# jinhan/tacotron2-vae

Hardware: AMD Instinct MI355X
Metric: mel-frames/s (train step, batch=6, 80-mel) (higher is better)
Workload: dtype f32; 1 GPU; configs[1]: Tacotron2-VAE fp32 train step (fwd+loss+bwd+clip+Adam), B=6/GPU fixed shape T_in=84 T_out=400, dropout on, random-init seed 1234; step_mode=hip-graph replay, decoder_forward=persistent, decoder_backward=persistent, startup_steps=43, global_batch=6, parallelism=dp1

## Files before the change

include/t2vae.h:

```cpp
#ifndef T2VAE_H
#define T2VAE_H
#include <stdint.h>
#ifdef __cplusplus
extern "C" {
#endif

#define T2V_OK 0
#define T2V_ERR_DIMS -1
#define T2V_ERR_ARG -2
#define T2V_ERR_LAUNCH -3

const char* t2v_version(void);
const char* t2v_last_error(void);

void t2v_set_phase_profile(unsigned long long* dev_buf32);
int t2v_stamp(unsigned long long* dev_buf, int slot, void* stream);
int t2v_debug_spin(int wgs, int microseconds, void* stream);

typedef struct t2v_step_params {
    uint64_t epoch;
    float lr;
    float bc1;
    float bc2s;
    float kl_weight;
// ... 165 lines not shown
    const float* proj_b;
    const float* prenet_w1;
} t2v_dec_persist_weights;
typedef struct t2v_dec_persist_bufs {
    const float* memory;
    const float* pm;
    const int32_t* lengths;
    const float* pre_first;
    float* MEL;
    float* GATE;
    float* AL;
    int32_t* stop_flag;
    void* exchange;
    uint32_t* err_word;
} t2v_dec_persist_bufs;
long t2v_decoder_persist_scratch_floats(int B, int t_end);
int t2v_decoder_persist_supported(int B, int T_in);
int t2v_decoder_infer_persistent(const t2v_dec_persist_weights* w, const t2v_dec_persist_bufs* s, int B, int T_in,
                                 int t_end, float gate_threshold, float p_prenet, uint64_t seed, void* stream);

typedef struct t2v_dec_items {
    int32_t* stop_item;
    const uint64_t* item_seeds;
} t2v_dec_items;
int t2v_decoder_infer_steps_items(const t2v_dec_weights* w, const t2v_dec_infer_bufs* s, int B, int T_in,
                                  int t_begin, int t_end, float gate_threshold, float p_prenet,
                                  int external_prenet, uint64_t seed, const t2v_dec_items* items, void* stream);
int t2v_decoder_infer_persistent_items(const t2v_dec_persist_weights* w, const t2v_dec_persist_bufs* s, int B, int T_in,
                                       int t_end, float gate_threshold, float p_prenet, uint64_t seed,
                                       const t2v_dec_items* items, void* stream);

int t2v_conv1d_stat_blocks(int B, int T, int Cin, int Cout, int KS);
int t2v_conv1d_stat_blocks_bf16(int B, int T, int Cin, int Cout, int KS);
int t2v_conv1d_fwd(const float* W, const float* X, const float* bias, float* Y, float* stat_part,
                   int B, int Cin, int T, int Cout, int KS, void* stream);
int t2v_conv1d_dw_scratch_floats(int B, int Cin, int T, int Cout, int KS);
int t2v_conv1d_bwd(const float* W, const float* X, const float* dY, float* dX, float* dW, float* Wt_scratch,
                   float* dw_scratch,
                   int B, int Cin, int T, int Cout, int KS, void* stream);
int t2v_conv1d_flip_weights(const float* const* W, float* const* Wt, const int* Cout, const int* Cin, int KS, int n,
                            void* stream);
int t2v_conv1d_fwd_bf16(const float* W, const float* X, const float* bias, float* Y, float* stat_part,
                        void* Wp_scratch, int B, int Cin, int T, int Cout, int KS, void* stream);
int t2v_conv1d_bwd_bf16(const float* W, const float* X, const float* dY, float* dX, float* dW,
                        void* Wp_scratch, float* dw_scratch, int B, int Cin, int T, int Cout, int KS, void* stream);

int t2v_bn_act_fwd(const float* y, const float* stat_part, int nblk, const float* gamma, const float* beta,
                   float* running_mean, float* running_var, float* mean_out, float* rstd_out, float* out,
                   int B, int M, int T, int act, int training, float p_drop, float momentum, float eps,
                   uint64_t seed, uint32_t rng_stream, uint32_t rng_t, void* stream);
int t2v_bn_act_fwd_len(const float* y, const float* gamma, const float* beta, const float* running_mean,
                       const float* running_var, float* out, const int32_t* lengths, int B, int M, int T, int act, float eps,
                       void* stream);
int t2v_bn_act_bwd(const float* y, const float* dout, const float* mean, const float* rstd,
                   const float* gamma, const float* beta, float* dy, float* dgamma, float* dbeta,
                   float* dconv_bias, int B, int M, int T, int act, float p_drop, uint64_t seed,
                   uint32_t rng_stream, uint32_t rng_t, void* stream);
int t2v_bn_act_bwd_eval(const float* y, const float* dout, const float* mean, const float* rstd,
                   const float* gamma, const float* beta, float* dy, float* dgamma, float* dbeta,
                   float* dconv_bias, int B, int M, int T, int act, float p_drop, uint64_t seed,
                   uint32_t rng_stream, uint32_t rng_t, void* stream);

int t2v_embedding_fwd(const long long* ids, const float* W, float* out_bct, int B, int T, int C, int n_symbols, void* stream);
int t2v_embedding_bwd(const long long* ids, const float* dy_bct, float* dW, int B, int T, int C, int n_symbols, void* stream);

int t2v_gemm_epilogue_bwd(const float* dy, const float* y, float* out, size_t n, float scale, void* stream);
// ... 198 lines not shown
```

tacotron2-vae_amd/csrc/conv_gemm.hip:

```cpp
#include <stdlib.h>
#include "t2v_common.h"
#include "t2v_kernels.h"
#include "t2v_coop.h"


#define CG_BM 64
#define CG_BN 64
#define CG_BK 32

struct ConvGemmArgs {
    const float* W;
    const float* X;
    const float* dY;
    const float* bias;
    float* Y;
    float* stat_part;
    int B, Cin, T, M, KS;
};

template <int MODE, int KS>
__global__ __launch_bounds__(256) void k_conv_gemm(ConvGemmArgs a) {
    __shared__ float As[2][CG_BK][CG_BM + 1];
    __shared__ float Bs[2][CG_BK][CG_BN + 1];
    __shared__ float red[2][CG_BM][2];
    const int tid = threadIdx.x, wave = tid >> 6, lane = tid & 63;
    const int wm = wave >> 1, wn = wave & 1;
    const int m0 = blockIdx.y * CG_BM, n0 = blockIdx.x * CG_BN;
    constexpr int P = KS >> 1;
    const int BT = a.B * a.T, CK = a.Cin * KS;
    const int Kdim = MODE == 0 ? CK : BT;
    const int Ndim = MODE == 0 ? BT : CK;

    constexpr int NE = CG_BM * CG_BK / 256;
    float ra[NE], rb[NE];
    int b_bb = 0, b_t = 0;
    bool b_nok = false;
// ... 95 lines not shown
                red[wn][ml][1] = q;
            }
        }
        __syncthreads();
        if (tid < CG_BM) {
            const int m = m0 + tid;
            if (m < a.M) {
                float* dst = a.stat_part + ((size_t)blockIdx.x * a.M + m) * 2;
                dst[0] = red[0][tid][0] + red[1][tid][0];
                dst[1] = red[0][tid][1] + red[1][tid][1];
            }
        }
    }
}

#define CT_BM 64
#define CT_AS 80
#define CT_KT 80

struct ConvTiledArgs {
    const float* W;
    const float* X;
    const float* dY;
    const float* bias;
    float* Y;
    float* stat_part;
    int B, Cin, T, M, tiles_per_item;
    unsigned long long* prof;
    float* ks_part;
    unsigned* ks_ctr;
};

template <int NTW>
__global__ __launch_bounds__(256) void k_conv5_fwd(ConvTiledArgs a) {
    constexpr int BN = 16 * NTW;
    constexpr int XW = BN + 4;
    constexpr int XS = BN == 32 ? 48 : BN <= 64 ? 80 : 112;
    constexpr int NX = (16 * XW + 255) / 256;
    __shared__ float As[2][CT_KT][CT_AS];
    __shared__ float Xs[2][16][XS];
    const int tid = threadIdx.x, wave = tid >> 6, lane = tid & 63;
    const int kq = lane >> 4, j = lane & 15;
    const int bb = blockIdx.x / a.tiles_per_item, t0 = (blockIdx.x % a.tiles_per_item) * BN;
    const int m0 = blockIdx.y * CT_BM;
    const int CK = a.Cin * 5;
    const int nkt_all = a.Cin / 16;
    const int kt0 = gridDim.z > 1 ? (int)blockIdx.z * (nkt_all / 2) : 0;
    const int nkt = gridDim.z > 1 ? (blockIdx.z == 0 ? nkt_all / 2 : nkt_all - nkt_all / 2) : nkt_all;

    const bool stamp = a.prof && tid == 0 && blockIdx.x == 0 && blockIdx.y == 0 && blockIdx.z == 0;
    if (stamp) { a.prof[0] = __builtin_readcyclecounter(); a.prof[2] = wall_clock64(); }
    float4 ra[5];
    float rx[NX];
    const int a_m = tid & 63, w4 = tid >> 6;
    const float* a_row = a.W + (size_t)min(m0 + a_m, a.M - 1) * CK + 4 * w4;
    int a_lds[20];
#pragma unroll
    for (int q = 0; q < 20; ++q) {
        const int k = 4 * w4 + 16 * (q >> 2) + (q & 3);
        const int c = k / 5, kx = k - 5 * c;
        a_lds[q] = (16 * kx + c) * CT_AS + a_m;
    }
    const float* x_item = a.X + (size_t)bb * a.Cin * a.T;
    int x_goff[NX], x_lds[NX];
    bool x_ok[NX];
#pragma unroll
// ... 35 lines not shown
    for (int q = 0; q < NSTORE; ++q) store_one(0, q);
    __syncthreads();
    for (int kt = 0; kt < nkt; ++kt) {
        const int buf = kt & 1;
        const int kn = min(kt + 1, nkt - 1);
        const float* ap = &As[buf][kq][16 * wave + j];
        const float* xp = &Xs[buf][kq][j];
        float av[2], bv[2][NTW];
        av[0] = ap[0];
#pragma unroll
        for (int n = 0; n < NTW; ++n) bv[0][n] = xp[16 * n];
#pragma unroll
        for (int s = 0; s < 20; ++s) {
            if (s < NLOAD) load_one(kn, s);
            if (s + 1 < 20) {
                av[(s + 1) & 1] = ap[4 * (s + 1) * CT_AS];
#pragma unroll
                for (int n = 0; n < NTW; ++n)
                    bv[(s + 1) & 1][n] = xp[4 * ((s + 1) & 3) * XS + 16 * n + ((s + 1) >> 2)];
            }
            __builtin_amdgcn_sched_barrier(0);
#pragma unroll
            for (int n = 0; n < NTW; ++n) acc[n] = mfma16x4(av[s & 1], bv[s & 1][n], acc[n]);
            __builtin_amdgcn_sched_barrier(0);
            if (s >= S_ST0) {
#pragma unroll
                for (int q = 3 * (s - S_ST0); q < 3 * (s - S_ST0) + 3; ++q) store_one(buf ^ 1, q);
                __builtin_amdgcn_sched_barrier(0);
            }
        }
        __syncthreads();
    }
    if (stamp) { a.prof[1] = __builtin_readcyclecounter(); a.prof[3] = wall_clock64(); }
    if (gridDim.z > 1) {
        const size_t tile = (size_t)blockIdx.y * gridDim.x + blockIdx.x, ntile = (size_t)gridDim.x * gridDim.y;
        float* mine = a.ks_part + ((blockIdx.z * ntile + tile) * 256 + tid) * (4 * NTW);
#pragma unroll
        for (int n = 0; n < NTW; ++n)
#pragma unroll
            for (int r = 0; r < 4; ++r) st_sc1(mine + 4 * n + r, acc[n][r]);
        __shared__ unsigned second_;
        asm volatile("s_waitcnt vmcnt(0)" ::: "memory");
        __syncthreads();
        if (tid == 0) second_ = __hip_atomic_fetch_add(a.ks_ctr + tile, 1u, __ATOMIC_RELAXED, __HIP_MEMORY_SCOPE_AGENT);
        __syncthreads();
        if (second_ == 0u) return;
        if (tid == 0) __hip_atomic_store(a.ks_ctr + tile, 0u, __ATOMIC_RELAXED, __HIP_MEMORY_SCOPE_AGENT);
        const float* other = a.ks_part + (((1 - blockIdx.z) * ntile + tile) * 256 + tid) * (4 * NTW);
        float o[NTW][4];
#pragma unroll
        for (int n = 0; n < NTW; ++n)
#pragma unroll
            for (int r = 0; r < 4; ++r) o[n][r] = ld_sc1(other + 4 * n + r);
#pragma unroll
        for (int n = 0; n < NTW; ++n)
#pragma unroll
            for (int r = 0; r < 4; ++r) acc[n][r] += o[n][r];
    }
    float psum[4] = {0.f, 0.f, 0.f, 0.f}, psq[4] = {0.f, 0.f, 0.f, 0.f};
#pragma unroll
    for (int r = 0; r < 4; ++r) {
        const int m = m0 + 16 * wave + 4 * kq + r;
        if (m < a.M) {
            const float bv = a.bias ? a.bias[m] : 0.f;
            float* yrow = a.Y + ((size_t)bb * a.M + m) * a.T;
#pragma unroll
            for (int n = 0; n < NTW; ++n) {
                const int t = t0 + 16 * n + j;
                if (t < a.T) {
                    const float v = acc[n][r] + bv;
                    yrow[t] = v;
                    psum[r] += v;
                    psq[r] = fmaf(v, v, psq[r]);
                }
            }
        }
    }
    if (a.stat_part) {
#pragma unroll
        for (int r = 0; r < 4; ++r) {
            const float s1 = row16_sum(psum[r]), s2 = row16_sum(psq[r]);
            const int m = m0 + 16 * wave + 4 * kq + r;
            if (j == 0 && m < a.M) {
                float* dst = a.stat_part + ((size_t)blockIdx.x * a.M + m) * 2;
                dst[0] = s1;
                dst[1] = s2;
            }
        }
    }
}

template <int BT>
__global__ __launch_bounds__(256) void k_conv5_dw(ConvTiledArgs a) {
    constexpr int XW = BT + 4;
    constexpr int XS = (BT == 80) ? 100 : 116;
    constexpr int NA = BT / 16;
    constexpr int NX = (16 * XW + 255) / 256;
    __shared__ float As[2][BT][CT_AS];
    __shared__ float Xs[2][16][XS];
    const int tid = threadIdx.x, wave = tid >> 6, lane = tid & 63;
    const int kq = lane >> 4, j = lane & 15;
    const int c0 = blockIdx.x * 16, m0 = blockIdx.y * CT_BM;
    const int CK = a.Cin * 5;
    const int tiles = (a.T + BT - 1) / BT, nkt_all = a.B * tiles;
    const int per = (nkt_all + gridDim.z - 1) / gridDim.z;
    const int kt_lo = blockIdx.z * per, kt_hi = min(nkt_all, kt_lo + per);
    const bool vec = (a.T & 3) == 0;

    float4 ra[NA];
    float rx[NX];
    const int a_m = tid & 63;
    const bool a_ok = m0 + a_m < a.M;
    auto load_tiles = [&](int kt) {
        const int bb = kt / tiles, t0 = (kt - bb * tiles) * BT;
        const float* arow = a.dY + ((size_t)bb * a.M + (a_ok ? m0 + a_m : 0)) * a.T;
#pragma unroll
        for (int i = 0; i < NA; ++i) {
            const int t = t0 + 4 * ((tid >> 6) + 4 * i);
            float4 v = make_float4(0.f, 0.f, 0.f, 0.f);
            if (a_ok) {
                if (vec) {
                    if (t < a.T) v = *(const float4*)(arow + t);
// ... 503 lines not shown
    for (int i = 0; i < 5; ++i) {
        const int bn = cands[i];
        const long wgs = (long)B * ((T + bn - 1) / bn) * ((M + CT_BM - 1) / CT_BM);
        const long cost = ((wgs + T2V_NWG - 1) / T2V_NWG) * (bn + 40);
        if (best_cost < 0 || cost < best_cost || (cost == best_cost && bn > best)) { best = bn; best_cost = cost; }
    }
    return best;
}
static inline int conv5_pick_bn_ks(int T, int B, int M, int Cin, int* ks) {
    static const int ksplit_on = getenv("T2V_CONV_KSPLIT") ? atoi(getenv("T2V_CONV_KSPLIT")) : 1;
    *ks = 1;
    const int bn1 = conv5_pick_bn(T, B, M);
    if (!ksplit_on || Cin < 256 || getenv("T2V_CONV_BN")) return bn1;
    const int cands[5] = {32, 48, 64, 80, 96};
    const long w1 = (long)B * ((T + bn1 - 1) / bn1) * ((M + CT_BM - 1) / CT_BM);
    long best_cost = 2 * ((w1 + T2V_NWG - 1) / T2V_NWG) * (bn1 + 40);
    int best = bn1;
    for (int i = 0; i < 5; ++i) {
        const int bn = cands[i];
        const long wgs = 2 * (long)B * ((T + bn - 1) / bn) * ((M + CT_BM - 1) / CT_BM);
        if (wgs > (ksplit_on == 2 ? 2 * T2V_NWG : T2V_NWG)) continue;
        const long cost = ((wgs + T2V_NWG - 1) / T2V_NWG) * ((bn + 40) + 16);
        if (cost < best_cost) { best = bn; best_cost = cost; *ks = 2; }
    }
    return best;
}
static inline bool conv5_tiled_ok(int Cin, int KS) { return KS == 5 && Cin % 16 == 0; }
bool t2v_conv5_x3_ok(int B, int Cin, int T, int Cout, int KS);
int t2v_conv5_x3_stat_blocks(int B, int T);
int t2v_conv5_x3_run(const float* W, const float* X, const float* bias, float* Y, float* stat_part, int B, int Cin, int T, int M,
                     hipStream_t stream, int np);
bool t2v_conv5_planes_bf16_ok(int B, int Cin, int T, int Cout, int KS);

static void launch_conv5_fwd(const float* W, const float* X, const float* bias, float* Y, float* stat_part, int B,
                             int Cin, int T, int M, hipStream_t stream) {
    int ks = 1;
    const int BN = conv5_pick_bn_ks(T, B, M, Cin, &ks);
    ConvTiledArgs a;
    a.W = W; a.X = X; a.dY = nullptr; a.bias = bias; a.Y = Y; a.stat_part = stat_part;
    a.B = B; a.Cin = Cin; a.T = T; a.M = M; a.tiles_per_item = (T + BN - 1) / BN;
    a.prof = g_t2v_prof;
    a.ks_part = nullptr; a.ks_ctr = nullptr;
    dim3 grid(B * a.tiles_per_item, (M + CT_BM - 1) / CT_BM);
    const long ntile = (long)grid.x * grid.y;
    if (ks == 2) {
        const size_t pf = (size_t)2 * ntile * 256 * 4 * (BN / 16);
        a.ks_part = conv_ks_scratch(pf);
        a.ks_ctr = a.ks_part ? t2v_arrival_counters((int)ntile) : nullptr;
        if (a.ks_part && a.ks_ctr) grid.z = 2; else a.ks_part = nullptr;
    }
    if (BN == 32) k_conv5_fwd<2><<<grid, 256, 0, stream>>>(a);
    else if (BN == 48) k_conv5_fwd<3><<<grid, 256, 0, stream>>>(a);
    else if (BN == 64) k_conv5_fwd<4><<<grid, 256, 0, stream>>>(a);
    else if (BN == 80) k_conv5_fwd<5><<<grid, 256, 0, stream>>>(a);
    else k_conv5_fwd<6><<<grid, 256, 0, stream>>>(a);
}

static void launch_conv5_fwd_bf16(const float* W, int flipT, unsigned short* Wp, const float* X, const float* bias,
                                  float* Y, float* stat_part, int B, int Cin, int T, int M, int W_M, int W_Cin,
                                  hipStream_t stream) {
    const size_t n = (size_t)W_M * W_Cin * 5;
    k_conv5_pack_bf16<<<(unsigned)((n + 255) / 256), 256, 0, stream>>>(W, Wp, W_M, W_Cin, flipT);
    int ks_unused = 1;
    const int BN = conv5_pick_bn_ks(T, B, M, Cin, &ks_unused);
    ConvBf16Args a;
    a.Wp = Wp; a.X = X; a.bias = bias; a.Y = Y; a.stat_part = stat_part;
    a.B = B; a.Cin = Cin; a.T = T; a.M = M; a.tiles_per_item = (T + BN - 1) / BN;
    dim3 grid(B * a.tiles_per_item, (M + CT_BM - 1) / CT_BM);
    static const int k32 = getenv("T2V_CONV_BF16_K32") ? atoi(getenv("T2V_CONV_BF16_K32")) : 1;
    if (k32 && Cin % 32 == 0) {
        if (BN == 32) k_conv5_fwd_bf16k32<2><<<grid, 256, 0, stream>>>(a);
        else if (BN == 48) k_conv5_fwd_bf16k32<3><<<grid, 256, 0, stream>>>(a);
        else if (BN == 64) k_conv5_fwd_bf16k32<4><<<grid, 256, 0, stream>>>(a);
        else if (BN == 80) k_conv5_fwd_bf16k32<5><<<grid, 256, 0, stream>>>(a);
        else k_conv5_fwd_bf16k32<6><<<grid, 256, 0, stream>>>(a);
        return;
    }
    if (BN == 32) k_conv5_fwd_bf16<2><<<grid, 256, 0, stream>>>(a);
    else if (BN == 48) k_conv5_fwd_bf16<3><<<grid, 256, 0, stream>>>(a);
    else if (BN == 64) k_conv5_fwd_bf16<4><<<grid, 256, 0, stream>>>(a);
    else if (BN == 80) k_conv5_fwd_bf16<5><<<grid, 256, 0, stream>>>(a);
    else k_conv5_fwd_bf16<6><<<grid, 256, 0, stream>>>(a);
// ... 177 lines not shown
```

tacotron2-vae_amd/csrc/t2v_x3.h:

```cpp
#pragma once
#include "t2v_common.h"

__device__ __forceinline__ void t2v_split8(const float (&v)[8], uint4& p0, uint4& p1, uint4& p2) {
    unsigned q0[4], q1[4], q2[4];
#pragma unroll
    for (int c = 0; c < 4; ++c) {
        const float x = v[2 * c], y = v[2 * c + 1];
        const unsigned h = t2v_pack_bf16x2(x, y);
        const float r1x = x - __uint_as_float(h << 16), r1y = y - __uint_as_float(h & 0xffff0000u);
        const unsigned m = t2v_pack_bf16x2(r1x, r1y);
        const float r2x = r1x - __uint_as_float(m << 16), r2y = r1y - __uint_as_float(m & 0xffff0000u);
        q0[c] = h; q1[c] = m; q2[c] = t2v_pack_bf16x2(r2x, r2y);
    }
    p0 = make_uint4(q0[0], q0[1], q0[2], q0[3]);
    p1 = make_uint4(q1[0], q1[1], q1[2], q1[3]);
    p2 = make_uint4(q2[0], q2[1], q2[2], q2[3]);
}

__device__ __forceinline__ void t2v_dma16(const void* gsrc, unsigned lds_addr) {
    unsigned keep;
    asm volatile("s_mov_b32 %0, m0\n\ts_mov_b32 m0, %2\n\ts_nop 0\n\tglobal_load_lds_dwordx4 %1, off\n\ts_mov_b32 m0, %0"
                 : "=&s"(keep) : "v"(gsrc), "s"(lds_addr) : "memory");
}

template <int N>
__device__ __forceinline__ void t2v_wait_vmcnt() {
    if constexpr (N == 0) asm volatile("s_waitcnt vmcnt(0)" ::: "memory");
    else if constexpr (N == 4) asm volatile("s_waitcnt vmcnt(4)" ::: "memory");
    else if constexpr (N == 6) asm volatile("s_waitcnt vmcnt(6)" ::: "memory");
    else if constexpr (N == 7) asm volatile("s_waitcnt vmcnt(7)" ::: "memory");
    else if constexpr (N == 8) asm volatile("s_waitcnt vmcnt(8)" ::: "memory");
    else if constexpr (N == 10) asm volatile("s_waitcnt vmcnt(10)" ::: "memory");
    else if constexpr (N == 12) asm volatile("s_waitcnt vmcnt(12)" ::: "memory");
    else if constexpr (N == 14) asm volatile("s_waitcnt vmcnt(14)" ::: "memory");
    else if constexpr (N == 16) asm volatile("s_waitcnt vmcnt(16)" ::: "memory");
    else static_assert(N == 0, "add the literal");
}
```

tacotron2-vae_amd/t2v_hip.py:

```python
import collections
import ctypes as C
import math
import os

import torch

_HERE = os.path.dirname(os.path.abspath(__file__))
_LIB_PATH = os.environ.get('T2V_LIB') or os.path.join(_HERE, 'libt2vae_hip.so')
_lib = None

H, E, PRE, A, F_LOC, KS, XW, KATT, KATT_INF, G4 = 1024, 512, 256, 128, 32, 31, 2560, 1536, 1792, 4096


class T2VHipError(RuntimeError):
    pass


class _DecWeights(C.Structure):
    _fields_ = [(n, C.c_void_p) for n in (
        'packF_att', 'packF_dec', 'packB_att', 'packB_dec', 'bias_att', 'bias_dec', 'wqT', 'wcomb', 'v')] + [
        ('packs_bf16', C.c_int32)]


class _DecTrainBufs(C.Structure):
# ... 17 lines not shown
        'memory', 'pm', 'lengths', 'pre_first', 'MEL', 'GATE', 'AL', 'stop_flag', 'exchange', 'err_word')]


class _DecTrainPersistWeights(C.Structure):
    C_NAME = 't2v_dec_train_persist_weights'
    _fields_ = [(n, C.c_void_p) for n in (
        'w_ih_att', 'w_hh_att', 'w_ih_dec', 'w_hh_dec', 'bias_dec', 'wq', 'wcomb', 'v')]


class _GemmGroup(C.Structure):
    C_NAME = 't2v_gemm_group'
    _fields_ = [('A', C.c_void_p), ('sAi', C.c_long), ('sAk', C.c_long), ('nb', C.c_int), ('B', C.c_void_p * 3), ('sBj', C.c_long * 3),
                ('sBk', C.c_long * 3), ('N', C.c_int * 3), ('C', C.c_void_p * 3), ('ldc', C.c_int * 3)]


class _AchainDw(C.Structure):
    C_NAME = 't2v_achain_dw'
    _fields_ = [('planes', C.c_void_p), ('d_w_ih', C.c_void_p), ('ld_ih', C.c_int), ('d_w_hh', C.c_void_p), ('ld_hh', C.c_int),
                ('accumulate', C.c_int), ('tile_cap', C.c_int)]


class _DecInferBufs(C.Structure):
    _fields_ = [(n, C.c_void_p) for n in (
        'memory', 'pm', 'lengths', 'XS', 'CA', 'CD', 'QP', 'AL', 'ACUM', 'PRE', 'MEL', 'GATE', 'stop_flag',
        'prenet_w1', 'proj_w', 'proj_b')]


class _DecItems(C.Structure):
    C_NAME = 't2v_dec_items'
    _fields_ = [(n, C.c_void_p) for n in ('stop_item', 'item_seeds')]


EXPORTS = ('t2v_version', 't2v_last_error', 't2v_stamp', 't2v_debug_spin', 't2v_pack_lstm_weights', 't2v_pack_lstm_weights_bf16', 't2v_decoder_train_fwd',
           't2v_decoder_train_bwd', 't2v_clip_adam_step', 't2v_clip_adam_step_guarded', 't2v_decoder_replay_fwd_kernels', 't2v_mel_frontend', 't2v_set_phase_profile', 't2v_decoder_infer_steps', 't2v_conv1d_stat_blocks', 't2v_conv1d_stat_blocks_bf16', 't2v_conv1d_fwd', 't2v_conv1d_bwd', 't2v_conv1d_fwd_bf16', 't2v_conv1d_bwd_bf16', 't2v_conv1d_dw_scratch_floats', 't2v_conv1d_flip_weights', 't2v_gemm_bf16', 't2v_gemm_bf16_splitk', 't2v_gemm_bf16_splitk_scratch_floats', 't2v_attn_wgrad', 't2v_attn_wgrad_scratch_floats',
           't2v_bn_act_fwd', 't2v_bn_act_bwd', 't2v_bn_act_bwd_eval', 't2v_bilstm_fwd', 't2v_bilstm_bwd', 't2v_gemm_f32', 't2v_conv2d_s2_fwd', 't2v_conv2d_s2_bwd', 't2v_conv2d_s2_dw_scratch_floats', 't2v_conv2d_s2_fwd_gemm', 't2v_conv2d_s2_bwd_gemm',
           't2v_conv2d_s2_gemm_scratch_floats',
           't2v_gru_fwd', 't2v_gru_bwd', 't2v_loss_fwd_bwd', 't2v_fuse_location_weights', 't2v_decoder_qp_floats',
           't2v_set_step_params', 't2v_set_step_params_stream', 't2v_decoder_replay_bwd_kernels', 't2v_embedding_fwd', 't2v_embedding_bwd', 't2v_gemm_f32_splitk', 't2v_gemm_splitk_scratch_floats', 't2v_gemm_f32_batched',
           't2v_decoder_infer_persistent', 't2v_decoder_persist_supported', 't2v_decoder_persist_scratch_floats',
           't2v_attn_bwd_slices', 't2v_colsum', 't2v_colsum_scratch_floats', 't2v_gemm_epilogue_bwd',
           't2v_decoder_train_fwd_persistent', 't2v_decoder_train_persist_supported',
           't2v_decoder_train_persist_scratch_floats', 't2v_decoder_bwd_persist_supported',
           't2v_decoder_bwd_achain_scratch_floats', 't2v_decoder_bwd_achain', 't2v_decoder_bwd_achain_prepare',
           't2v_decoder_bwd_achain_prepared', 't2v_decoder_bwd_persist_slices', 't2v_decoder_bwd_achain_dq_offset',
           't2v_decoder_bwd_achain_dw_offset', 't2v_gemm_f32_grouped_handed', 't2v_gemm_f32_grouped_group_offset', 't2v_mask_outputs', 't2v_reparam_fwd',
           't2v_reparam_bwd', 't2v_gather_words', 't2v_concat2_rows',
           't2v_decoder_train_fwd_persistent16', 't2v_decoder_train_persist16_supported',
           't2v_decoder_train_persist16_scratch_floats', 't2v_decoder_bwd_persistent16', 't2v_decoder_bwd_persist16_supported',
           't2v_decoder_bwd_persist16_scratch_floats', 't2v_decoder_bwd_persist16_dq_offset', 't2v_decoder_bwd_persist16_slices',
           't2v_decoder_bwd_persist16_fits', 't2v_gemm_f32_set_mode', 't2v_conv1d_x3_set_mode', 't2v_gemm_f32_grouped',
           't2v_gemm_f32_grouped_scratch_floats', 't2v_gemm_bf16_grouped', 't2v_gemm_bf16_grouped_scratch_floats',
           't2v_decoder_bwd_persistent16_prepare', 't2v_decoder_bwd_persistent16_prepared',
           't2v_stft_polar', 't2v_istft', 't2v_istft_scratch_bytes', 't2v_griffin_lim', 't2v_griffin_lim_scratch_bytes',
           't2v_mel_to_magnitude', 't2v_decoder_infer_steps_items', 't2v_decoder_infer_persistent_items', 't2v_bn_act_fwd_len',
           't2v_mask_time', 't2v_conv2d_s2_fwd_ragged', 't2v_conv2d_s2_fwd_gemm_ragged', 't2v_conv2d_s2_gemm_ragged_scratch_floats',
           't2v_gru_fwd_len', 't2v_mel_dtw', 't2v_mel_dtw_scratch_bytes', 't2v_tsne_scratch_bytes', 't2v_tsne_affinities',
           't2v_tsne_gradient', 't2v_tsne_run', 't2v_f0_yin', 't2v_alignment_stats', 't2v_alignment_scratch_bytes',
           't2v_mel_to_magnitude_nnls', 't2v_griffin_lim_fast', 't2v_griffin_lim_fast_scratch_bytes',
           't2v_resample', 't2v_trim_bounds', 't2v_crop_rows', 't2v_latent_scratch_bytes', 't2v_latent_neighbours',
           't2v_mel_cepstrum', 't2v_cep_dtw_scratch_bytes', 't2v_cep_dtw_path', 't2v_cep_dtw_forward', 't2v_cep_dtw_walk',
           't2v_path_scores', 't2v_loudness', 't2v_loudness_scratch_bytes', 't2v_scale_rows')


def lib_path():
    return _LIB_PATH


# ... 124 lines not shown
    lib.t2v_mel_dtw_scratch_bytes.argtypes = [C.c_int, C.c_int, C.c_int]
    lib.t2v_mel_dtw_scratch_bytes.restype = C.c_size_t
    lib.t2v_mel_dtw.argtypes = [vp, vp, C.c_int, vp, vp, C.c_int, C.c_int, C.c_int, vp, vp, vp]
    lib.t2v_mel_cepstrum.argtypes = [vp, vp, C.c_int, C.c_int, C.c_int, C.c_int, vp, vp, C.c_int, vp]
    lib.t2v_cep_dtw_scratch_bytes.argtypes = [C.c_int, C.c_int, C.c_int]
    lib.t2v_cep_dtw_scratch_bytes.restype = C.c_size_t
    lib.t2v_cep_dtw_forward.argtypes = [vp, vp, C.c_int, vp, vp, C.c_int, C.c_int, C.c_int, vp, vp, vp]
    lib.t2v_cep_dtw_walk.argtypes = [vp, C.c_int, vp, C.c_int, C.c_int, vp, vp, vp, C.c_int, vp]
    lib.t2v_cep_dtw_path.argtypes = [vp, vp, C.c_int, vp, vp, C.c_int, C.c_int, C.c_int, vp, vp, vp, C.c_int, vp, vp]
    lib.t2v_path_scores.argtypes = [vp, vp, C.c_int, vp, vp, C.c_int, vp, vp, C.c_int, vp, C.c_int, vp, C.c_int, C.c_int, C.c_int,
                                    vp, vp, vp]
    lib.t2v_tsne_scratch_bytes.argtypes = [C.c_int, C.c_int]
    lib.t2v_tsne_scratch_bytes.restype = C.c_size_t
    lib.t2v_tsne_affinities.argtypes = [vp, C.c_int, C.c_int, C.c_float, vp, vp, vp]
    lib.t2v_tsne_gradient.argtypes = [vp, vp, C.c_int, C.c_float, vp, vp, vp, vp]
    lib.t2v_tsne_run.argtypes = [vp, vp, C.c_int, C.c_int, C.c_float, vp, vp, vp]
    lib.t2v_f0_yin.argtypes = [vp, vp, C.c_int, C.c_int, C.c_int, C.c_int, C.c_float, vp, vp, C.c_int, vp]
    lib.t2v_latent_scratch_bytes.argtypes = [C.c_int] * 5
    lib.t2v_latent_scratch_bytes.restype = C.c_size_t
    lib.t2v_latent_neighbours.argtypes = [vp, vp, C.c_int, C.c_int, C.c_int, vp, C.c_int, vp, vp, C.c_int, C.c_int] + [vp] * 7
    lib.t2v_resample.argtypes = [vp, C.c_int, C.c_float, vp, C.c_int, C.c_int, vp, C.c_int, C.c_int, C.c_int, vp, C.c_int, vp]
    lib.t2v_trim_bounds.argtypes = [vp, vp, C.c_int, C.c_int, C.c_float, C.c_int, vp, C.c_int, vp, vp]
    lib.t2v_crop_rows.argtypes = [vp, C.c_int, vp, C.c_int, vp, C.c_int, C.c_int, vp, vp]
    lib.t2v_loudness_scratch_bytes.argtypes = [C.c_int, C.c_int, C.c_int]
    lib.t2v_loudness_scratch_bytes.restype = C.c_size_t
    lib.t2v_loudness.argtypes = [vp, vp, C.c_int, C.c_int, vp, C.c_int, vp, C.c_int, vp, C.c_int, vp, vp, vp]
    lib.t2v_scale_rows.argtypes = [vp, vp, C.c_int, C.c_int, vp, vp]
    lib.t2v_alignment_scratch_bytes.argtypes = [C.c_int, C.c_int, C.c_int]
    lib.t2v_alignment_scratch_bytes.restype = C.c_size_t
    lib.t2v_alignment_stats.argtypes = [vp, C.c_longlong, C.c_longlong, vp, vp, C.c_int, C.c_int, C.c_int, C.c_int, C.c_float, vp,
                                        C.c_int, vp, C.c_int, vp, vp, vp, vp]
    lib.t2v_conv1d_stat_blocks.argtypes = [C.c_int, C.c_int, C.c_int, C.c_int, C.c_int]
    lib.t2v_conv1d_stat_blocks_bf16.argtypes = [C.c_int, C.c_int, C.c_int, C.c_int, C.c_int]
    lib.t2v_conv1d_fwd.argtypes = [vp, vp, vp, vp, vp, C.c_int, C.c_int, C.c_int, C.c_int, C.c_int, vp]
    lib.t2v_conv1d_bwd.argtypes = [vp, vp, vp, vp, vp, vp, vp, C.c_int, C.c_int, C.c_int, C.c_int, C.c_int, vp]
    lib.t2v_conv1d_dw_scratch_floats.argtypes = [C.c_int] * 5
    lib.t2v_conv1d_flip_weights.argtypes = [vp, vp, vp, vp, C.c_int, C.c_int, vp]
    lib.t2v_conv1d_fwd_bf16.argtypes = [vp, vp, vp, vp, vp, vp, C.c_int, C.c_int, C.c_int, C.c_int, C.c_int, vp]
    lib.t2v_conv1d_bwd_bf16.argtypes = [vp, vp, vp, vp, vp, vp, vp, C.c_int, C.c_int, C.c_int, C.c_int, C.c_int, vp]
    lib.t2v_bn_act_fwd.argtypes = [vp, vp, C.c_int, vp, vp, vp, vp, vp, vp, vp, C.c_int, C.c_int, C.c_int, C.c_int,
                                   C.c_int, C.c_float, C.c_float, C.c_float, C.c_uint64, C.c_uint32, C.c_uint32, vp]
    lib.t2v_bn_act_bwd.argtypes = [vp, vp, vp, vp, vp, vp, vp, vp, vp, vp, C.c_int, C.c_int, C.c_int, C.c_int, C.c_float,
                                   C.c_uint64, C.c_uint32, C.c_uint32, vp]
    lib.t2v_bn_act_bwd_eval.argtypes = lib.t2v_bn_act_bwd.argtypes
    lib.t2v_bn_act_fwd_len.argtypes = [vp, vp, vp, vp, vp, vp, vp, C.c_int, C.c_int, C.c_int, C.c_int, C.c_float, vp]
    lib.t2v_mask_time.argtypes = [vp, vp, vp, C.c_int, C.c_int, C.c_int, vp]
    lib.t2v_bilstm_fwd.argtypes = [vp, vp, vp, vp, vp, vp, vp, vp, C.c_int, C.c_int, vp]
    lib.t2v_bilstm_bwd.argtypes = [vp, vp, vp, vp, vp, vp, vp, vp, C.c_int, C.c_int, vp]
    lib.t2v_gemm_f32.argtypes = [vp, C.c_long, C.c_long, vp, C.c_long, C.c_long, vp, vp, C.c_int, C.c_int, C.c_int,
                                 C.c_int, C.c_int, C.c_int, C.c_float, C.c_uint64, C.c_uint32, C.c_uint32, vp]
    lib.t2v_gemm_bf16.argtypes = lib.t2v_gemm_f32.argtypes
    lib.t2v_gemm_bf16_splitk.argtypes = lib.t2v_gemm_f32.argtypes[:-1] + [vp, vp]
    lib.t2v_gemm_bf16_splitk_scratch_floats.argtypes = [C.c_int, C.c_int, C.c_int]
    lib.t2v_gemm_bf16_splitk_scratch_floats.restype = C.c_long
    lib.t2v_gemm_f32_splitk.argtypes = lib.t2v_gemm_f32.argtypes[:-1] + [vp, vp]
    lib.t2v_gemm_f32_batched.argtypes = [vp, C.c_long, C.c_long, C.c_long, vp, C.c_long, C.c_long, C.c_long, vp, C.c_long,
                                         C.c_int, C.c_int, C.c_int, C.c_int, C.c_int, vp]
    lib.t2v_gemm_splitk_scratch_floats.argtypes = [C.c_int, C.c_int, C.c_int]
    lib.t2v_gemm_splitk_scratch_floats.restype = C.c_long
    lib.t2v_attn_wgrad.argtypes = [vp, vp, vp, vp, vp, vp, vp, vp, C.c_int, C.c_int, C.c_int, vp]
    lib.t2v_attn_wgrad_scratch_floats.argtypes = []
    lib.t2v_conv2d_s2_fwd.argtypes = [vp, vp, vp, vp, C.c_int, C.c_int, C.c_int, C.c_int, C.c_int, C.c_int, vp]
    lib.t2v_conv2d_s2_bwd.argtypes = [vp, vp, vp, vp, vp, vp, C.c_int, C.c_int, C.c_int, C.c_int, C.c_int, C.c_int, vp]
    lib.t2v_conv2d_s2_fwd_gemm.argtypes = [vp, vp, vp, vp, vp, C.c_int, C.c_int, C.c_int, C.c_int, C.c_int, C.c_int, vp]
    lib.t2v_conv2d_s2_bwd_gemm.argtypes = [vp, vp, vp, vp, vp, vp, C.c_int, C.c_int, C.c_int, C.c_int, C.c_int, C.c_int, vp]
    lib.t2v_conv2d_s2_gemm_scratch_floats.argtypes = [C.c_int] * 6
# ... 2543 lines not shown
```

Measured before the change: 228,200 mel-frames/s.

## Stage conv5 forward tiles via direct global-to-LDS loads with three-stage ring

```diff
diff --git a/include/t2vae.h b/include/t2vae.h
--- a/include/t2vae.h
+++ b/include/t2vae.h
@@ -221,6 +221,7 @@
 
 int t2v_conv1d_stat_blocks(int B, int T, int Cin, int Cout, int KS);
 int t2v_conv1d_stat_blocks_bf16(int B, int T, int Cin, int Cout, int KS);
+long long t2v_conv1d_staged_launches(void);
 int t2v_conv1d_fwd(const float* W, const float* X, const float* bias, float* Y, float* stat_part,
                    int B, int Cin, int T, int Cout, int KS, void* stream);
 int t2v_conv1d_dw_scratch_floats(int B, int Cin, int T, int Cout, int KS);
diff --git a/tacotron2-vae_amd/csrc/conv_gemm.hip b/tacotron2-vae_amd/csrc/conv_gemm.hip
--- a/tacotron2-vae_amd/csrc/conv_gemm.hip
+++ b/tacotron2-vae_amd/csrc/conv_gemm.hip
@@ -1,7 +1,9 @@
 #include <stdlib.h>
+#include <type_traits>
 #include "t2v_common.h"
 #include "t2v_kernels.h"
 #include "t2v_coop.h"
+#include "t2v_x3.h"
 
 
 #define CG_BM 64
@@ -163,6 +165,68 @@
 };
 
 template <int NTW>
+__device__ __forceinline__ void conv5_fwd_finish(const ConvTiledArgs& a, f32x4 (&acc)[NTW], int bb, int t0, int m0) {
+    const int tid = threadIdx.x, wave = tid >> 6, lane = tid & 63;
+    const int kq = lane >> 4, j = lane & 15;
+    if (gridDim.z > 1) {
+        const size_t tile = (size_t)blockIdx.y * gridDim.x + blockIdx.x, ntile = (size_t)gridDim.x * gridDim.y;
+        float* mine = a.ks_part + ((blockIdx.z * ntile + tile) * 256 + tid) * (4 * NTW);
+#pragma unroll
+        for (int n = 0; n < NTW; ++n)
+#pragma unroll
+            for (int r = 0; r < 4; ++r) st_sc1(mine + 4 * n + r, acc[n][r]);
+        __shared__ unsigned second_;
+        asm volatile("s_waitcnt vmcnt(0)" ::: "memory");
+        __syncthreads();
+        if (tid == 0) second_ = __hip_atomic_fetch_add(a.ks_ctr + tile, 1u, __ATOMIC_RELAXED, __HIP_MEMORY_SCOPE_AGENT);
+        __syncthreads();
+        if (second_ == 0u) return;
+        if (tid == 0) __hip_atomic_store(a.ks_ctr + tile, 0u, __ATOMIC_RELAXED, __HIP_MEMORY_SCOPE_AGENT);
+        const float* other = a.ks_part + (((1 - blockIdx.z) * ntile + tile) * 256 + tid) * (4 * NTW);
+        float o[NTW][4];
+#pragma unroll
+        for (int n = 0; n < NTW; ++n)
+#pragma unroll
+            for (int r = 0; r < 4; ++r) o[n][r] = ld_sc1(other + 4 * n + r);
+#pragma unroll
+        for (int n = 0; n < NTW; ++n)
+#pragma unroll
+            for (int r = 0; r < 4; ++r) acc[n][r] += o[n][r];
+    }
+    float psum[4] = {0.f, 0.f, 0.f, 0.f}, psq[4] = {0.f, 0.f, 0.f, 0.f};
+#pragma unroll
+    for (int r = 0; r < 4; ++r) {
+        const int m = m0 + 16 * wave + 4 * kq + r;
+        if (m < a.M) {
+            const float bv = a.bias ? a.bias[m] : 0.f;
+            float* yrow = a.Y + ((size_t)bb * a.M + m) * a.T;
+#pragma unroll
+            for (int n = 0; n < NTW; ++n) {
+                const int t = t0 + 16 * n + j;
+                if (t < a.T) {
+                    const float v = acc[n][r] + bv;
+                    yrow[t] = v;
+                    psum[r] += v;
+                    psq[r] = fmaf(v, v, psq[r]);
+                }
+            }
+        }
+    }
+    if (a.stat_part) {
+#pragma unroll
+        for (int r = 0; r < 4; ++r) {
+            const float s1 = row16_sum(psum[r]), s2 = row16_sum(psq[r]);
+            const int m = m0 + 16 * wave + 4 * kq + r;
+            if (j == 0 && m < a.M) {
+                float* dst = a.stat_part + ((size_t)blockIdx.x * a.M + m) * 2;
+                dst[0] = s1;
+                dst[1] = s2;
+            }
+        }
+    }
+}
+
+template <int NTW>
 __global__ __launch_bounds__(256) void k_conv5_fwd(ConvTiledArgs a) {
     constexpr int BN = 16 * NTW;
     constexpr int XW = BN + 4;
@@ -264,62 +328,124 @@
         __syncthreads();
     }
     if (stamp) { a.prof[1] = __builtin_readcyclecounter(); a.prof[3] = wall_clock64(); }
-    if (gridDim.z > 1) {
-        const size_t tile = (size_t)blockIdx.y * gridDim.x + blockIdx.x, ntile = (size_t)gridDim.x * gridDim.y;
-        float* mine = a.ks_part + ((blockIdx.z * ntile + tile) * 256 + tid) * (4 * NTW);
-#pragma unroll
-        for (int n = 0; n < NTW; ++n)
-#pragma unroll
-            for (int r = 0; r < 4; ++r) st_sc1(mine + 4 * n + r, acc[n][r]);
-        __shared__ unsigned second_;
-        asm volatile("s_waitcnt vmcnt(0)" ::: "memory");
-        __syncthreads();
-        if (tid == 0) second_ = __hip_atomic_fetch_add(a.ks_ctr + tile, 1u, __ATOMIC_RELAXED, __HIP_MEMORY_SCOPE_AGENT);
-        __syncthreads();
-        if (second_ == 0u) return;
-        if (tid == 0) __hip_atomic_store(a.ks_ctr + tile, 0u, __ATOMIC_RELAXED, __HIP_MEMORY_SCOPE_AGENT);
-        const float* other = a.ks_part + (((1 - blockIdx.z) * ntile + tile) * 256 + tid) * (4 * NTW);
-        float o[NTW][4];
-#pragma unroll
-        for (int n = 0; n < NTW; ++n)
-#pragma unroll
-            for (int r = 0; r < 4; ++r) o[n][r] = ld_sc1(other + 4 * n + r);
-#pragma unroll
-        for (int n = 0; n < NTW; ++n)
-#pragma unroll
-            for (int r = 0; r < 4; ++r) acc[n][r] += o[n][r];
-    }
-    float psum[4] = {0.f, 0.f, 0.f, 0.f}, psq[4] = {0.f, 0.f, 0.f, 0.f};
-#pragma unroll
-    for (int r = 0; r < 4; ++r) {
-        const int m = m0 + 16 * wave + 4 * kq + r;
-        if (m < a.M) {
-            const float bv = a.bias ? a.bias[m] : 0.f;
-            float* yrow = a.Y + ((size_t)bb * a.M + m) * a.T;
+    conv5_fwd_finish<NTW>(a, acc, bb, t0, m0);
+}
+
+#define CD_RING 3
+#define CD_AS 84
+__device__ float g_conv5_zero[4];
+
+template <int NTW>
+__global__ __launch_bounds__(256) void k_conv5_fwd_dma(ConvTiledArgs a) {
+    constexpr int BN = 16 * NTW;
+    constexpr int XW = BN + 4;
+    constexpr int XS = BN == 32 ? 48 : BN <= 64 ? 80 : 112;
+    constexpr int NXD = 16 * XS / 256;
+    constexpr int G = 6 + NXD;
+    constexpr int AST = CT_BM * CD_AS, STG = AST + 16 * XS;
+    static_assert(16 * XS % 256 == 0 && AST % 256 == 0, "whole 64-lane requests");
+    __shared__ __attribute__((aligned(16))) float lds_[CD_RING * STG];
+    const unsigned lds0 = (unsigned)(unsigned long)(__attribute__((address_space(3))) void*)&lds_[0];
+    const int tid = threadIdx.x, wave = __builtin_amdgcn_readfirstlane(tid >> 6), lane = tid & 63;
+    const int kq = lane >> 4, j = lane & 15;
+    const int bb = blockIdx.x / a.tiles_per_item, t0 = (blockIdx.x % a.tiles_per_item) * BN;
+    const int m0 = blockIdx.y * CT_BM;
+    const int CK = a.Cin * 5;
+    const int nkt_all = a.Cin / 16;
+    const int kt0 = gridDim.z > 1 ? (int)blockIdx.z * (nkt_all / 2) : 0;
+    const int nkt = gridDim.z > 1 ? (blockIdx.z == 0 ? nkt_all / 2 : nkt_all - nkt_all / 2) : nkt_all;
+
+    const bool stamp = a.prof && tid == 0 && blockIdx.x == 0 && blockIdx.y == 0 && blockIdx.z == 0;
+    if (stamp) { a.prof[0] = __builtin_readcyclecounter(); a.prof[2] = wall_clock64(); }
+    const float* a_ptr[6];
+#pragma unroll
+    for (int i = 0; i < 6; ++i) {
+        const int u = 64 * min(wave + 4 * i, 20) + lane;
+        const int row = u / 21, pc = u - 21 * row;
+        a_ptr[i] = a.W + (size_t)min(m0 + row, a.M - 1) * CK + 80 * kt0 + 4 * min(pc, 19);
+    }
+    const float* x_ptr[NXD];
+    size_t x_step[NXD];
+#pragma unroll
+    for (int i = 0; i < NXD; ++i) {
+        const int e = 64 * (wave + 4 * i) + lane;
+        const int c = e / XS, jj = e - c * XS;
+        const int t = t0 - 2 + jj;
+        const bool ok = jj < XW && t >= 0 && t < a.T;
+        x_ptr[i] = ok ? a.X + ((size_t)bb * a.Cin + 16 * kt0 + c) * a.T + t : g_conv5_zero;
+        x_step[i] = ok ? (size_t)16 * a.T : 0;
+    }
+    auto request = [&](unsigned dst, int q) {
+        if (q < 5) {
+            t2v_dma16(a_ptr[q], dst + 1024u * (unsigned)wave + 4096u * q);
+            a_ptr[q] += 80;
+        } else if (q == 5) {
+            t2v_dma16(a_ptr[5], dst + 20480u);
+            a_ptr[5] += 80;
+        } else if (q < G) {
+            t2v_dma4(x_ptr[q - 6], dst + 4u * AST + 256u * (unsigned)wave + 1024u * (q - 6));
+            x_ptr[q - 6] += x_step[q - 6];
+        }
+    };
+
+    f32x4 acc[NTW];
+#pragma unroll
+    for (int n = 0; n < NTW; ++n) acc[n] = f32x4{0.f, 0.f, 0.f, 0.f};
+#pragma unroll
+    for (int q = 0; q < G; ++q) request(lds0, q);
+    if (nkt > 1) {
+#pragma unroll
+        for (int q = 0; q < G; ++q) request(lds0 + 4u * STG, q);
+    }
+    if (nkt > 1) t2v_wait_vmcnt<G>(); else t2v_wait_vmcnt<0>();
+    __syncthreads();
+    constexpr int CD_SYNC = 10;
+    constexpr int TWO = G > 20 - CD_SYNC ? G - (20 - CD_SYNC) : 0;
+    static_assert(G <= 2 * (20 - CD_SYNC) && (TWO == 0 || NTW >= 3), "a tile's requests fit the steps behind the barrier");
+    const int lane_a = CD_AS * (16 * wave + j) + 5 * kq, lane_x = AST + kq * XS + j;
+    float av[2], bv[2][NTW];
+    auto fetch = [&](const float* ap, const float* xp, int s) {
+        av[s & 1] = ap[20 * (s & 3) + (s >> 2)];
+#pragma unroll
+        for (int n = 0; n < NTW; ++n) bv[s & 1][n] = xp[4 * (s & 3) * XS + 16 * n + (s >> 2)];
+    };
+    auto tile = [&](auto more_c, const float* ap, const float* xp, const float* ap1, const float* xp1, unsigned dst2) {
+        constexpr bool MORE = decltype(more_c)::value;
+#pragma unroll
+        for (int s = 0; s < 20; ++s) {
+            if (s == CD_SYNC) {
+                t2v_wait_vmcnt<0>();
+                __syncthreads();
+                __builtin_amdgcn_sched_barrier(0);
+            }
+            const int sr = s - CD_SYNC;
+            const int q0 = !MORE || sr < 0 ? -1 : sr < TWO ? 2 * sr : sr + TWO;
+            const int q1 = MORE && sr >= 0 && sr < TWO ? 2 * sr + 1 : -1;
 #pragma unroll
             for (int n = 0; n < NTW; ++n) {
-                const int t = t0 + 16 * n + j;
-                if (t < a.T) {
-                    const float v = acc[n][r] + bv;
-                    yrow[t] = v;
-                    psum[r] += v;
-                    psq[r] = fmaf(v, v, psq[r]);
-                }
-            }
-        }
-    }
-    if (a.stat_part) {
-#pragma unroll
-        for (int r = 0; r < 4; ++r) {
-            const float s1 = row16_sum(psum[r]), s2 = row16_sum(psq[r]);
-            const int m = m0 + 16 * wave + 4 * kq + r;
-            if (j == 0 && m < a.M) {
-                float* dst = a.stat_part + ((size_t)blockIdx.x * a.M + m) * 2;
-                dst[0] = s1;
-                dst[1] = s2;
-            }
-        }
-    }
+                acc[n] = mfma16x4(av[s & 1], bv[s & 1][n], acc[n]);
+                __builtin_amdgcn_sched_barrier(0);
+                if (n == 0) { if (s + 1 < 20) fetch(ap, xp, s + 1); else fetch(ap1, xp1, 0); }
+                if (n == 1 && q0 >= 0 && q0 < G) request(dst2, q0);
+                if (n == 2 && q1 >= 0) request(dst2, q1);
+                __builtin_amdgcn_sched_barrier(0);
+            }
+        }
+    };
+    fetch(&lds_[lane_a], &lds_[lane_x], 0);
+    int stg = 0;
+    for (int kt = 0; kt < nkt; ++kt) {
+        const int stg1 = stg == CD_RING - 1 ? 0 : stg + 1, stg2 = stg == 0 ? CD_RING - 1 : stg - 1;
+        const float* ap = &lds_[stg * STG + lane_a];
+        const float* xp = &lds_[stg * STG + lane_x];
+        const float* ap1 = &lds_[stg1 * STG + lane_a];
+        const float* xp1 = &lds_[stg1 * STG + lane_x];
+        if (kt + 2 < nkt) tile(std::true_type{}, ap, xp, ap1, xp1, lds0 + 4u * (unsigned)(stg2 * STG));
+        else tile(std::false_type{}, ap, xp, ap1, xp1, 0u);
+        stg = stg1;
+    }
+    if (stamp) { a.prof[1] = __builtin_readcyclecounter(); a.prof[3] = wall_clock64(); }
+    conv5_fwd_finish<NTW>(a, acc, bb, t0, m0);
 }
 
 template <int BT>
@@ -889,6 +1015,9 @@
                      hipStream_t stream, int np);
 bool t2v_conv5_planes_bf16_ok(int B, int Cin, int T, int Cout, int KS);
 
+static std::atomic<long long> g_conv5_staged_launches{0};
+extern "C" long long t2v_conv1d_staged_launches(void) { return g_conv5_staged_launches.load(std::memory_order_relaxed); }
+
 static void launch_conv5_fwd(const float* W, const float* X, const float* bias, float* Y, float* stat_part, int B,
                              int Cin, int T, int M, hipStream_t stream) {
     int ks = 1;
@@ -905,6 +1034,16 @@
         a.ks_part = conv_ks_scratch(pf);
         a.ks_ctr = a.ks_part ? t2v_arrival_counters((int)ntile) : nullptr;
         if (a.ks_part && a.ks_ctr) grid.z = 2; else a.ks_part = nullptr;
+    }
+    static const int staging = getenv("T2V_CONV_STAGING") ? atoi(getenv("T2V_CONV_STAGING")) : 1;
+    if (staging && ((size_t)W & 15) == 0) {
+        g_conv5_staged_launches.fetch_add(1, std::memory_order_relaxed);
+        if (BN == 32) k_conv5_fwd_dma<2><<<grid, 256, 0, stream>>>(a);
+        else if (BN == 48) k_conv5_fwd_dma<3><<<grid, 256, 0, stream>>>(a);
+        else if (BN == 64) k_conv5_fwd_dma<4><<<grid, 256, 0, stream>>>(a);
+        else if (BN == 80) k_conv5_fwd_dma<5><<<grid, 256, 0, stream>>>(a);
+        else k_conv5_fwd_dma<6><<<grid, 256, 0, stream>>>(a);
+        return;
     }
     if (BN == 32) k_conv5_fwd<2><<<grid, 256, 0, stream>>>(a);
     else if (BN == 48) k_conv5_fwd<3><<<grid, 256, 0, stream>>>(a);
diff --git a/tacotron2-vae_amd/csrc/t2v_x3.h b/tacotron2-vae_amd/csrc/t2v_x3.h
--- a/tacotron2-vae_amd/csrc/t2v_x3.h
+++ b/tacotron2-vae_amd/csrc/t2v_x3.h
@@ -23,6 +23,12 @@
                  : "=&s"(keep) : "v"(gsrc), "s"(lds_addr) : "memory");
 }
 
+__device__ __forceinline__ void t2v_dma4(const void* gsrc, unsigned lds_addr) {
+    unsigned keep;
+    asm volatile("s_mov_b32 %0, m0\n\ts_mov_b32 m0, %2\n\ts_nop 0\n\tglobal_load_lds_dword %1, off\n\ts_mov_b32 m0, %0"
+                 : "=&s"(keep) : "v"(gsrc), "s"(lds_addr) : "memory");
+}
+
 template <int N>
 __device__ __forceinline__ void t2v_wait_vmcnt() {
     if constexpr (N == 0) asm volatile("s_waitcnt vmcnt(0)" ::: "memory");
@@ -30,8 +36,11 @@
     else if constexpr (N == 6) asm volatile("s_waitcnt vmcnt(6)" ::: "memory");
     else if constexpr (N == 7) asm volatile("s_waitcnt vmcnt(7)" ::: "memory");
     else if constexpr (N == 8) asm volatile("s_waitcnt vmcnt(8)" ::: "memory");
+    else if constexpr (N == 9) asm volatile("s_waitcnt vmcnt(9)" ::: "memory");
     else if constexpr (N == 10) asm volatile("s_waitcnt vmcnt(10)" ::: "memory");
+    else if constexpr (N == 11) asm volatile("s_waitcnt vmcnt(11)" ::: "memory");
     else if constexpr (N == 12) asm volatile("s_waitcnt vmcnt(12)" ::: "memory");
+    else if constexpr (N == 13) asm volatile("s_waitcnt vmcnt(13)" ::: "memory");
     else if constexpr (N == 14) asm volatile("s_waitcnt vmcnt(14)" ::: "memory");
     else if constexpr (N == 16) asm volatile("s_waitcnt vmcnt(16)" ::: "memory");
     else static_assert(N == 0, "add the literal");
diff --git a/tacotron2-vae_amd/t2v_hip.py b/tacotron2-vae_amd/t2v_hip.py
--- a/tacotron2-vae_amd/t2v_hip.py
+++ b/tacotron2-vae_amd/t2v_hip.py
@@ -73,7 +73,7 @@
 
 
 EXPORTS = ('t2v_version', 't2v_last_error', 't2v_stamp', 't2v_debug_spin', 't2v_pack_lstm_weights', 't2v_pack_lstm_weights_bf16', 't2v_decoder_train_fwd',
-           't2v_decoder_train_bwd', 't2v_clip_adam_step', 't2v_clip_adam_step_guarded', 't2v_decoder_replay_fwd_kernels', 't2v_mel_frontend', 't2v_set_phase_profile', 't2v_decoder_infer_steps', 't2v_conv1d_stat_blocks', 't2v_conv1d_stat_blocks_bf16', 't2v_conv1d_fwd', 't2v_conv1d_bwd', 't2v_conv1d_fwd_bf16', 't2v_conv1d_bwd_bf16', 't2v_conv1d_dw_scratch_floats', 't2v_conv1d_flip_weights', 't2v_gemm_bf16', 't2v_gemm_bf16_splitk', 't2v_gemm_bf16_splitk_scratch_floats', 't2v_attn_wgrad', 't2v_attn_wgrad_scratch_floats',
+           't2v_decoder_train_bwd', 't2v_clip_adam_step', 't2v_clip_adam_step_guarded', 't2v_decoder_replay_fwd_kernels', 't2v_mel_frontend', 't2v_set_phase_profile', 't2v_decoder_infer_steps', 't2v_conv1d_stat_blocks', 't2v_conv1d_stat_blocks_bf16', 't2v_conv1d_staged_launches', 't2v_conv1d_fwd', 't2v_conv1d_bwd', 't2v_conv1d_fwd_bf16', 't2v_conv1d_bwd_bf16', 't2v_conv1d_dw_scratch_floats', 't2v_conv1d_flip_weights', 't2v_gemm_bf16', 't2v_gemm_bf16_splitk', 't2v_gemm_bf16_splitk_scratch_floats', 't2v_attn_wgrad', 't2v_attn_wgrad_scratch_floats',
            't2v_bn_act_fwd', 't2v_bn_act_bwd', 't2v_bn_act_bwd_eval', 't2v_bilstm_fwd', 't2v_bilstm_bwd', 't2v_gemm_f32', 't2v_conv2d_s2_fwd', 't2v_conv2d_s2_bwd', 't2v_conv2d_s2_dw_scratch_floats', 't2v_conv2d_s2_fwd_gemm', 't2v_conv2d_s2_bwd_gemm',
            't2v_conv2d_s2_gemm_scratch_floats',
            't2v_gru_fwd', 't2v_gru_bwd', 't2v_loss_fwd_bwd', 't2v_fuse_location_weights', 't2v_decoder_qp_floats',
@@ -264,6 +264,8 @@
                                         C.c_int, vp, C.c_int, vp, vp, vp, vp]
     lib.t2v_conv1d_stat_blocks.argtypes = [C.c_int, C.c_int, C.c_int, C.c_int, C.c_int]
     lib.t2v_conv1d_stat_blocks_bf16.argtypes = [C.c_int, C.c_int, C.c_int, C.c_int, C.c_int]
+    lib.t2v_conv1d_staged_launches.argtypes = []
+    lib.t2v_conv1d_staged_launches.restype = C.c_longlong
     lib.t2v_conv1d_fwd.argtypes = [vp, vp, vp, vp, vp, C.c_int, C.c_int, C.c_int, C.c_int, C.c_int, vp]
     lib.t2v_conv1d_bwd.argtypes = [vp, vp, vp, vp, vp, vp, vp, C.c_int, C.c_int, C.c_int, C.c_int, C.c_int, vp]
     lib.t2v_conv1d_dw_scratch_floats.argtypes = [C.c_int] * 5
```

Result: faster. 230,900 mel-frames/s (median of 6 runs) (+1.2%).
